# Tangshitao/Semi-supervised-Adaptive-Distillation

Measured on AMD Instinct MI355X. Metric: images/sec (student+teacher fwd + student bwd) R50-FPN distill, 1/2/4/8 MI355X, higher is better.
Workload: dtype f32

## Files before the change

include/ssad_kernels.h:

```cpp
#ifndef SSAD_KERNELS_H_
#define SSAD_KERNELS_H_

#include <stddef.h>
#include <stdint.h>

#ifdef __cplusplus
extern "C" {
#endif

#define SSAD_API __attribute__((visibility("default")))

#define SSAD_E_BADARG (-1)
#define SSAD_E_WORKSPACE (-2)
#define SSAD_MAX_LEVELS 8
#define SSAD_MAX_CONV_PROBLEMS 24
#define SSAD_MAX_POWSUM_INPUTS 8

typedef void* ssad_stream_t;


typedef struct {
  float gamma;
  float alpha;
  float beta;
// ... 226 lines not shown
  float* out;
} ssad_image_norm;
SSAD_API size_t ssad_image_blobs_workspace_bytes(int N, int Hb, int Wb);
SSAD_API int ssad_image_blobs(
    const unsigned char* src, size_t src_bytes, const long long* offset_host, const int* h_host,
    const int* w_host, const int* out_h_host, const int* out_w_host, const double* scale_host,
    const int* flipped_host, int N, int Hb, int Wb, const ssad_image_norm* norms_host, int n_norms,
    void* workspace, size_t workspace_bytes, ssad_stream_t stream);


SSAD_API int ssad_conv_out_size(int in, int kernel, int dilation, int pad_a, int pad_b, int stride);
SSAD_API int ssad_im2col(const float* x, int C, int H, int W, int kh, int kw, int dil_h, int dil_w,
                         int pad_t, int pad_l, int pad_b, int pad_r, int stride_h, int stride_w,
                         float* col, ssad_stream_t stream);
SSAD_API int ssad_im2col_batched(const float* x, int N, int C, int H, int W, int kernel, int stride,
                                 int pad, float* col, ssad_stream_t stream);
SSAD_API int ssad_col2im(const float* col, int C, int H, int W, int kh, int kw, int dil_h,
                         int dil_w, int pad_t, int pad_l, int pad_b, int pad_r, int stride_h,
                         int stride_w, float* x, ssad_stream_t stream);
SSAD_API int ssad_channel_sum(const float* dy, int N, int C, int HW, float* out, int accumulate,
                              ssad_stream_t stream);
SSAD_API int ssad_relu_grad_rowsum(const float* y, const float* dy, float* dx, float* rowsum, int N,
                                   int C, int HW, ssad_stream_t stream);
SSAD_API int ssad_conv1x1_bias_act(const float* x, const float* w, const float* bias,
                                   const float* residual, float* y, int N, int C, int P, int M,
                                   int relu, ssad_stream_t stream);
SSAD_API int ssad_conv1x1_bias_act2(const float* x, int C1, const float* x2, int C2, const float* w,
                                    const float* bias, const float* residual, float* y, int N, int P,
                                    int M, int relu, ssad_stream_t stream);
#define SSAD_GEMM_RELU 1
#define SSAD_GEMM_ACCUMULATE 8
typedef struct ssad_gemm_conv {
  const float* a;
  const float* x;
  float* y;
  const float* bias;
  const float* residual;
  const float* mask;
  int lda, N, K, P, M, flags;
} ssad_gemm_conv;
SSAD_API int ssad_conv1x1_gemm(const ssad_gemm_conv* desc_host, ssad_stream_t stream);
SSAD_API size_t ssad_conv1x1_gemm_split_workspace_bytes(const ssad_gemm_conv* desc_host);
SSAD_API int ssad_conv1x1_gemm_split(const ssad_gemm_conv* desc_host, void* workspace, size_t workspace_bytes,
                                     ssad_stream_t stream);
SSAD_API int ssad_conv1x1_gemm_split_amax(const ssad_gemm_conv* desc_host, const float* packed_a, const unsigned* x_amax,
                                          unsigned* y_amax_out, void* workspace, size_t workspace_bytes,
                                          ssad_stream_t stream);
typedef struct ssad_gemm_pack_entry {
  const float* a;
  float* dst;
  int lda, K, M;
} ssad_gemm_pack_entry;
SSAD_API size_t ssad_gemm_split_filter_floats(int K, int M);
SSAD_API int ssad_gemm_split_pack_filters(const ssad_gemm_pack_entry* entries_host, int n_entries, ssad_stream_t stream);
SSAD_API int ssad_conv_implicit_gemm(const ssad_gemm_conv* d, int C, int H, int W, int kernel, int stride, int pad,
                                     ssad_stream_t stream);
SSAD_API size_t ssad_conv_implicit_gemm_workspace_bytes(int N, int M, int C, int H, int W, int kernel, int stride,
                                                        int pad);
SSAD_API int ssad_conv_implicit_gemm_ws(const ssad_gemm_conv* d, int C, int H, int W, int kernel, int stride, int pad,
                                        void* workspace, size_t workspace_bytes, ssad_stream_t stream);
SSAD_API size_t ssad_conv_kxk_wgrad_workspace_bytes(int N, int C, int H, int W, int M, int kernel, int stride,
                                                    int pad);
SSAD_API int ssad_conv_kxk_wgrad(const float* x, const float* dy, int N, int C, int H, int W, int M, int kernel,
                                 int stride, int pad, float* dw, int accumulate, void* workspace,
                                 size_t workspace_bytes, ssad_stream_t stream);
SSAD_API size_t ssad_conv_kxk_dgrad_workspace_bytes(int N, int C, int H, int W, int M, int kernel, int stride,
                                                    int pad);
SSAD_API int ssad_conv_kxk_dgrad(const float* w, const float* dy, int N, int C, int H, int W, int M, int kernel,
                                 int stride, int pad, float* dx, const float* mask, int accumulate, void* workspace,
                                 size_t workspace_bytes, ssad_stream_t stream);
SSAD_API int ssad_transpose_filter(const float* w, int M, int K, int ldm, float* wt, ssad_stream_t stream);
#define SSAD_MAX_TRANSPOSE_ENTRIES 64
typedef struct ssad_transpose_entry {
  const float* w;
  float* wt;
  int M, K, ldm;
  int reserved;
} ssad_transpose_entry;
SSAD_API int ssad_transpose_filters(const ssad_transpose_entry* entries_host, int n_entries, ssad_stream_t stream);
SSAD_API size_t ssad_conv1x1_wgrad_workspace_bytes(int N, int C, int P, int M);
SSAD_API int ssad_conv1x1_wgrad(const float* x, const float* dy, int N, int C, int P, int M, float* dw,
                                int accumulate, void* workspace, size_t workspace_bytes,
                                ssad_stream_t stream);
SSAD_API size_t ssad_conv1x1_wgrad_split_workspace_bytes(int N, int C, int P, int M);
SSAD_API int ssad_conv1x1_wgrad_split(const float* x, const float* dy, int N, int C, int P, int M, float* dw,
                                      int accumulate, void* workspace, size_t workspace_bytes,
                                      ssad_stream_t stream);
SSAD_API int ssad_conv1x1_wgrad_split_amax(const float* x, const float* dy, int N, int C, int P, int M, float* dw,
                                           int accumulate, void* workspace, size_t workspace_bytes,
                                           const unsigned* x_amax, const unsigned* dy_amax, ssad_stream_t stream);
SSAD_API int ssad_subsample(const float* x, int N, int C, int H, int W, int stride, float* y,
                            ssad_stream_t stream);
SSAD_API int ssad_subsample_grad(const float* dy, int N, int C, int H, int W, int stride, int accumulate,
                                 float* dx, ssad_stream_t stream);
SSAD_API long long ssad_grouped_conv3x3_filter_floats(int C, int group);
SSAD_API int ssad_grouped_conv3x3_pack_filter(const float* w, int C, int group, float* packed,
                                              ssad_stream_t stream);
SSAD_API int ssad_grouped_conv3x3_forward(const float* x, const float* packed, const float* bias, int N, int C,
                                          int H, int W, int group, int stride, int relu, float* y,
                                          ssad_stream_t stream);
SSAD_API int ssad_max_pool_forward(const float* x, int N, int C, int H, int W, int kh, int kw,
                                   int stride_h, int stride_w, int pad_t, int pad_l, int pad_b,
                                   int pad_r, float* y, ssad_stream_t stream);
SSAD_API int ssad_max_pool3x3s2_bias_relu(const float* x, const float* bias, int N, int C, int H,
                                          int W, int relu, float* y, ssad_stream_t stream);
SSAD_API int ssad_max_pool_backward(const float* x, const float* y, const float* dy, int N, int C,
// ... 203 lines not shown
```

semi-supervised-adaptive-distillation_amd/csrc/kernels/gemm_split.hip:

```cpp
#include <stdlib.h>

#include <mutex>

#include "split_common.h"

namespace {

using namespace ssad_split;

constexpr int PT = 128;
constexpr int MT = 256;
constexpr int HDR = 16;

__host__ __device__ constexpr int cdiv(int a, int b) { return (a + b - 1) / b; }

__global__ __launch_bounds__(kThreads) void gsplit_pack_a_kernel(const float* __restrict__ a, int lda, int K, int M,
                                                                 const unsigned* __restrict__ amax, float* __restrict__ dst) {
  const int KB = (K + 7) >> 3;
  const long long slots = (long long)KB * M;
  const float s = pow2f(15 - split_exponent(amax[0]));
  if (blockIdx.x == 0 && threadIdx.x < HDR) reinterpret_cast<unsigned*>(dst)[threadIdx.x] = threadIdx.x == 0 ? amax[0] : 0u;
  uint4* out = reinterpret_cast<uint4*>(dst + HDR);
  for (long long i = (long long)blockIdx.x * kThreads + threadIdx.x; i < slots; i += (long long)gridDim.x * kThreads) {
    const int m = (int)(i % M), kb = (int)(i / M);
// ... 6 lines not shown
    out[slots + i] = __builtin_bit_cast(uint4, lo);
  }
}

struct GPackTable {
  ssad_gemm_pack_entry e[SSAD_MAX_PACK_ENTRIES];
  int count;
};
__global__ __launch_bounds__(kThreads) void gsplit_zero_kernel(const GPackTable t) {
  for (int i = (int)threadIdx.x; i < t.count * HDR; i += kThreads) reinterpret_cast<unsigned*>(t.e[i / HDR].dst)[i % HDR] = 0u;
}
__global__ __launch_bounds__(kThreads) void gsplit_amax_kernel(const GPackTable t) {
  const ssad_gemm_pack_entry& E = t.e[blockIdx.y];
  unsigned m = 0;
  for (int k = (int)blockIdx.x; k < E.K; k += (int)gridDim.x)
    for (int j = (int)threadIdx.x; j < E.M; j += kThreads) {
      const unsigned a = __float_as_uint(E.a[(long long)k * E.lda + j]) & 0x7fffffffu;
      m = m > a ? m : a;
    }
#pragma unroll
  for (int o = 32; o > 0; o >>= 1) {
    const unsigned other = (unsigned)__shfl_xor((int)m, o, 64);
    m = m > other ? m : other;
  }
  __shared__ unsigned red[kThreads / 64];
  if ((threadIdx.x & 63) == 0) red[threadIdx.x >> 6] = m;
  __syncthreads();
  if (threadIdx.x == 0) {
    for (int w = 1; w < kThreads / 64; ++w) m = m > red[w] ? m : red[w];
    if (m) atomicMax(reinterpret_cast<unsigned*>(E.dst), m);
  }
}
__global__ __launch_bounds__(kThreads) void gsplit_pack_multi_kernel(const GPackTable t) {
  const ssad_gemm_pack_entry& E = t.e[blockIdx.y];
  const int KB = (E.K + 7) >> 3;
  const long long slots = (long long)KB * E.M;
  const float s = pow2f(15 - split_exponent(reinterpret_cast<const unsigned*>(E.dst)[0]));
  uint4* out = reinterpret_cast<uint4*>(E.dst + HDR);
  for (long long i = (long long)blockIdx.x * kThreads + threadIdx.x; i < slots; i += (long long)gridDim.x * kThreads) {
    const int m = (int)(i % E.M), kb = (int)(i / E.M);
    float v[8];
#pragma unroll
    for (int j = 0; j < 8; ++j) v[j] = kb * 8 + j < E.K ? E.a[(long long)(kb * 8 + j) * E.lda + m] : 0.0f;
    half8 hi, lo;
    split8(v, s, hi, lo);
    out[i] = __builtin_bit_cast(uint4, hi);
    out[slots + i] = __builtin_bit_cast(uint4, lo);
  }
}

#ifndef GFLY_ABLATE
#define GFLY_ABLATE 0
#endif
constexpr int FKC = 32;
constexpr int FWG = 512;
constexpr int F_XP = (FKC / 8) * PT * 16;
constexpr int F_WP = (FKC / 8) * MT * 16;
constexpr int F_STAGE = 2 * F_XP + 2 * F_WP;
constexpr int F_LDS = 2 * F_STAGE;

struct FArgs {
  const float* x;
  const float* ap;
  float* y;
  const float* bias;
  const float* residual;
  const float* mask;
  const unsigned* amax;
  unsigned* amax_out;
  int N, K, P, M, relu, accumulate;
  int ptiles, mblocks, items;
};

__global__ __launch_bounds__(FWG, 1) void gemm_fly_kernel(const FArgs q) {
  extern __shared__ __attribute__((aligned(16))) char flds[];
  const int tid = threadIdx.x, lane = tid & 63;
  const int wave = __builtin_amdgcn_readfirstlane(tid >> 6);
  const int wm = wave & 3, wp = wave >> 2;
  const int j = lane & 31, h = lane >> 5;
  const int K = q.K, M = q.M, P = q.P;
  const int KB = (K + 7) >> 3;
  const int nchunks = (K + FKC - 1) / FKC;

  int n, p0, ocb;
  {
    const int it = (int)blockIdx.x;
    const int xcd = it & 7, seq = it >> 3;
    const int mb = seq % q.mblocks;
    const int t = (seq / q.mblocks) * 8 + xcd;
    if (t >= q.N * q.ptiles) return;
    n = t / q.ptiles;
    p0 = (t - n * q.ptiles) * PT;
    ocb = mb * MT;
  }
  const unsigned w_lo_off = (unsigned)((long long)KB * M * 16);
  const __amdgpu_buffer_rsrc_t xrs = uniform_rsrc(q.x, (unsigned)((long long)q.N * K * P * 4));
  const __amdgpu_buffer_rsrc_t wrs = uniform_rsrc(q.ap + HDR, 2u * w_lo_off);
  const float sx = pow2f(15 - split_exponent(q.amax[0]));

  float xv[8];
  f32x4 wv[4];
  const int fpx = tid & (PT - 1), fkg = tid >> 7;
  const int fco = tid & (MT - 1), fkq = tid >> 8;
  const unsigned xbase = p0 + fpx < P ? (unsigned)((((long long)n * K + 8 * fkg) * P + p0 + fpx) * 4) : kOob;
  const int P4 = P * 4;
  auto fetch = [&](int c) {
    const int soff = __builtin_amdgcn_readfirstlane(c * FKC * P4);
#pragma unroll
    for (int e = 0; e < 8; ++e)
      xv[e] = __builtin_bit_cast(float, __builtin_amdgcn_raw_buffer_load_b32(
          xrs, c * FKC + 8 * fkg + e < K ? xbase : kOob, soff + e * P4, 0));
#pragma unroll
    for (int i = 0; i < 2; ++i) {
      const int kb = c * (FKC / 8) + fkq + 2 * i;
      const unsigned vo = (kb < KB && ocb + fco < M) ? (unsigned)((kb * M + ocb + fco) * 16) : kOob;
      wv[2 * i] = __builtin_bit_cast(f32x4, __builtin_amdgcn_raw_buffer_load_b128(wrs, vo, 0, 0));
      wv[2 * i + 1] = __builtin_bit_cast(f32x4, __builtin_amdgcn_raw_buffer_load_b128(wrs, vo, (int)w_lo_off, 0));
    }
  };
  auto put = [&](char* stage) {
    half8 hi, lo;
    split8(xv, sx, hi, lo);
    char* px = stage + (fkg * PT + fpx) * 16;
    *reinterpret_cast<half8*>(px) = hi;
    *reinterpret_cast<half8*>(px + F_XP) = lo;
#pragma unroll
    for (int i = 0; i < 2; ++i) {
      char* pw = stage + 2 * F_XP + ((fkq + 2 * i) * MT + fco) * 16;
      *reinterpret_cast<f32x4*>(pw) = wv[2 * i];
      *reinterpret_cast<f32x4*>(pw + F_WP) = wv[2 * i + 1];
    }
  };

  float16v acc[2][2];
#pragma unroll
  for (int i = 0; i < 2; ++i)
#pragma unroll
    for (int tt = 0; tt < 2; ++tt)
#pragma unroll
      for (int r = 0; r < 16; ++r) acc[i][tt][r] = 0.0f;

  auto step = [&](const char* stage, int st) {
    half8 ah[2], al[2], bh[2], bl[2];
    const int kg = 2 * st + h;
#pragma unroll
    for (int i = 0; i < 2; ++i) {
      const char* pw = stage + 2 * F_XP + (kg * MT + wm * 64 + i * 32 + j) * 16;
      ah[i] = *reinterpret_cast<const half8*>(pw);
      al[i] = *reinterpret_cast<const half8*>(pw + F_WP);
      const char* px = stage + (kg * PT + wp * 64 + i * 32 + j) * 16;
      bh[i] = *reinterpret_cast<const half8*>(px);
      bl[i] = *reinterpret_cast<const half8*>(px + F_XP);
    }
#pragma unroll
    for (int pr = 0; pr < ((GFLY_ABLATE & 8) ? 0 : (GFLY_ABLATE & 4) ? 1 : 3); ++pr)
#pragma unroll
      for (int i = 0; i < 2; ++i)
#pragma unroll
        for (int tt = 0; tt < 2; ++tt)
          acc[i][tt] = __builtin_amdgcn_mfma_f32_32x32x16_f16(pr == 1 ? al[i] : ah[i], pr == 2 ? bl[tt] : bh[tt],
                                                              acc[i][tt], 0, 0, 0);
    if (GFLY_ABLATE & 8) {
#pragma unroll
      for (int i = 0; i < 2; ++i) { acc[i][0][0] += (float)ah[i][0] + (float)al[i][1]; acc[i][1][0] += (float)bh[i][0] + (float)bl[i][1]; }
    }
  };

  fetch(0);
  put(flds);
  fetch(1);
  __syncthreads();
  for (int c = 0; c < nchunks; ++c) {
    const char* stage = flds + (c & 1) * F_STAGE;
    char* other = flds + ((c & 1) ^ 1) * F_STAGE;
    __builtin_amdgcn_sched_barrier(0);
    step(stage, 0);
    if (!(GFLY_ABLATE & 2)) put(other);
    __builtin_amdgcn_sched_barrier(0);
    if (!(GFLY_ABLATE & 1)) fetch(c + 2);
    __builtin_amdgcn_sched_barrier(0);
    step(stage, 1);
    __syncthreads();
  }

  const int oc_w = ocb + wm * 64;
  unsigned pvo[2];
#pragma unroll
  for (int tt = 0; tt < 2; ++tt) {
    const int px = p0 + wp * 64 + 32 * tt + j;
    pvo[tt] = px < P ? (unsigned)((((long long)n * M + 4 * h) * P + px) * 4) : kOob;
  }
  const int e2 = split_exponent(q.amax[0]) + split_exponent(reinterpret_cast<const unsigned*>(q.ap)[0]) - 30;
  const bool one_scale = e2 >= -126 && e2 <= 127;
  const float sc1 = one_scale ? pow2f(e2) : pow2f(split_exponent(q.amax[0]) - 15);
  const float sc2 = one_scale ? 1.0f : pow2f(split_exponent(reinterpret_cast<const unsigned*>(q.ap)[0]) - 15);
  const unsigned ybytes = (unsigned)((long long)q.N * M * P * 4);
  const __amdgpu_buffer_rsrc_t yrs = uniform_rsrc(q.y, ybytes);
  const __amdgpu_buffer_rsrc_t rrs = uniform_rsrc(q.residual ? (const void*)q.residual : (const void*)q.y, q.residual ? ybytes : 0u);
  const __amdgpu_buffer_rsrc_t mrs = uniform_rsrc(q.mask ? (const void*)q.mask : (const void*)q.y, q.mask ? ybytes : 0u);
  const __amdgpu_buffer_rsrc_t brs = uniform_rsrc(q.bias ? (const void*)q.bias : (const void*)q.y, q.bias ? (unsigned)M * 4u : 0u);
  const bool relu = q.relu, has_res = q.residual != nullptr, has_mask = q.mask != nullptr, accum = q.accumulate;
  const bool ragged = (M & 7) != 0;
  unsigned ymax = 0;
#pragma unroll
  for (int i = 0; i < 2; ++i) {
    const int oc0 = oc_w + i * 32;
    float4 bq[4];
#pragma unroll
    for (int g = 0; g < 4; ++g)
      bq[g] = __builtin_bit_cast(float4, __builtin_amdgcn_raw_buffer_load_b128(brs, (unsigned)h * 16u, (oc0 + 8 * g) * 4, 0));
#pragma unroll
    for (int tt = 0; tt < 2; ++tt) {
      float rs[16], mk[16], old[16];
#pragma unroll
      for (int r = 0; r < 16; ++r) {
        const int ch = oc0 + 8 * (r >> 2) + (r & 3);
        const unsigned vo = (ch < M && (!ragged || ch + 4 * h < M)) ? pvo[tt] : kOob;
        rs[r] = has_res ? __builtin_bit_cast(float, __builtin_amdgcn_raw_buffer_load_b32(rrs, vo, ch * P4, 0)) : 0.0f;
        mk[r] = has_mask ? __builtin_bit_cast(float, __builtin_amdgcn_raw_buffer_load_b32(mrs, vo, ch * P4, 0)) : 1.0f;
        old[r] = accum ? __builtin_bit_cast(float, __builtin_amdgcn_raw_buffer_load_b32(yrs, vo, ch * P4, 0)) : 0.0f;
      }
#pragma unroll
      for (int g = 0; g < 4; ++g) {
        if (oc0 + 8 * g >= M) continue;
#pragma unroll
        for (int e = 0; e < 4; ++e) {
          const int r = 4 * g + e;
          float v = one_scale ? fmaf(acc[i][tt][r], sc1, bq[g][e]) : acc[i][tt][r] * sc1 * sc2 + bq[g][e];
          v += rs[r];
          if (relu) v = fmaxf(v, 0.0f);
          if (has_mask) v = mk[r] > 0.0f ? v : 0.0f;
          v += old[r];
          const unsigned vo = (!ragged || oc0 + 8 * g + 4 * h + e < M) ? pvo[tt] : kOob;
          __builtin_amdgcn_raw_buffer_store_b32(__builtin_bit_cast(unsigned, v), yrs, vo, (oc0 + 8 * g + e) * P4, 0);
          const unsigned av = __builtin_bit_cast(unsigned, v) & 0x7fffffffu;
          if (vo != kOob) ymax = ymax > av ? ymax : av;
        }
      }
    }
  }
  if (q.amax_out) {
#pragma unroll
    for (int o = 32; o > 0; o >>= 1) {
      const unsigned other = (unsigned)__shfl_xor((int)ymax, o, 64);
      ymax = ymax > other ? ymax : other;
    }
    __syncthreads();
    unsigned* red = reinterpret_cast<unsigned*>(flds);
    if (lane == 0) red[wave] = ymax;
    __syncthreads();
    if (tid == 0) {
      for (int w = 1; w < FWG / 64; ++w) ymax = ymax > red[w] ? ymax : red[w];
      if (ymax) atomicMax(q.amax_out, ymax);
    }
  }
}

constexpr int WT = 256;
constexpr int WPX = 32;
constexpr int W_PL = (WPX / 8) * WT * 16;
constexpr int W_STAGE = 4 * W_PL;
constexpr int W_LDS = 2 * W_STAGE;

struct WPArgs {
  const float* x;
  const float* dy;
  float* slabs;
  const unsigned* xa;
  const unsigned* da;
  int N, C, P, M;
  int mtiles, ctiles, shares, per_share, total, cpi;
  int xcd_runs;
};

__global__ __launch_bounds__(FWG, 1) void wpoint_split_kernel(const WPArgs q) {
  extern __shared__ __attribute__((aligned(16))) char wlds[];
  const int tid = threadIdx.x, lane = tid & 63;
  const int wave = __builtin_amdgcn_readfirstlane(tid >> 6);
  const int wm = wave & 1, wc = wave >> 1;
  const int j = lane & 31, h = lane >> 5;
  const int P = q.P;

  const int tiles = q.mtiles * q.ctiles;
  int share, tile;
  if (q.xcd_runs) {
    const int xcd = blockIdx.x & 7, jj = blockIdx.x >> 3;
    share = xcd * q.xcd_runs + jj / tiles;
    tile = jj % tiles;
  } else {
    share = blockIdx.x / tiles;
    tile = blockIdx.x % tiles;
  }
  const int m0 = (tile / q.ctiles) * WT, c0 = (tile % q.ctiles) * WT;
  const int q_begin = share * q.per_share;
  const int q_end = q_begin + q.per_share < q.total ? q_begin + q.per_share : q.total;

  const __amdgpu_buffer_rsrc_t xrs = uniform_rsrc(q.x, (unsigned)((long long)q.N * q.C * P * 4));
  const __amdgpu_buffer_rsrc_t drs = uniform_rsrc(q.dy, (unsigned)((long long)q.N * q.M * P * 4));
  const float sx = pow2f(15 - split_exponent(q.xa[0]));
  const float sd = pow2f(15 - split_exponent(q.da[0]));

  float dv[2][8], xv[2][8];
  const int fpg = tid & 3, fch = tid >> 2;
  auto fetch = [&](int ck) {
    const int n = __builtin_amdgcn_readfirstlane(ck / q.cpi);
    const int p = (ck - n * q.cpi) * WPX + 8 * fpg;
    const bool pok = ck < q.total && p < P;
#pragma unroll
// ... 99 lines not shown
                                                            float* __restrict__ dw, int accumulate) {
  const long long e = (long long)blockIdx.x * 256 + threadIdx.x;
  if (e >= (long long)M * C) return;
  const int m = (int)(e / C), c = (int)(e - (long long)m * C);
  const float* p = slabs + (long long)m * Cp + c;
  const long long stride = (long long)Mp * Cp;
  float s = 0.0f;
  for (int sh = 0; sh < shares; ++sh) s += p[sh * stride];
  s = (s * pow2f(split_exponent(xa[0]) - 15)) * pow2f(split_exponent(da[0]) - 15);
  dw[e] = accumulate ? dw[e] + s : s;
}

int wpoint_plan(int N, int C, int P, int M, WPArgs* a) {
  if (N <= 0 || C <= 0 || P <= 0 || M <= 0 || (P & 7)) return SSAD_E_BADARG;
  if ((long long)N * C * P * 4 >= (1LL << 31) || (long long)N * M * P * 4 >= (1LL << 31)) return SSAD_E_BADARG;
  a->N = N; a->C = C; a->P = P; a->M = M;
  a->mtiles = cdiv(M, WT); a->ctiles = cdiv(C, WT);
  a->cpi = cdiv(P, WPX);
  a->total = N * a->cpi;
  const int cus = ssad_cu_count(), tiles = a->mtiles * a->ctiles;
  int s = cus / tiles;
  if (s < 1) s = 1;
  if (s >= 8) s &= ~7;
  while (s > 1 && a->total / s < 4) --s;
  a->per_share = cdiv(a->total, s);
  a->shares = cdiv(a->total, a->per_share);
  a->xcd_runs = (a->shares % 8 == 0) ? a->shares / 8 : 0;
  return 0;
}

struct GPlan {
  size_t amax_off, a_off, total;
};
int make_plan(const ssad_gemm_conv* d, GPlan* p) {
  if (!d || d->N <= 0 || d->K <= 0 || d->P <= 0 || d->M <= 0 || d->lda < d->M) return SSAD_E_BADARG;
  const int KB = (d->K + 7) >> 3;
  const long long aslots = (long long)KB * d->M;
  if ((long long)d->N * d->K * d->P * 4 >= (1LL << 31) || (long long)d->N * d->M * d->P * 4 >= (1LL << 31) ||
      aslots * 32 >= (1LL << 31))
    return SSAD_E_BADARG;
  p->amax_off = 0;
  p->a_off = 256;
  p->total = p->a_off + (size_t)HDR * 4 + (size_t)aslots * 32;
  return 0;
}

}

extern "C" {

size_t ssad_conv1x1_gemm_split_workspace_bytes(const ssad_gemm_conv* d) {
  GPlan p;
  return make_plan(d, &p) ? 0 : p.total;
}

size_t ssad_gemm_split_filter_floats(int K, int M) {
  if (K <= 0 || M <= 0) return 0;
  return (size_t)HDR + (size_t)((K + 7) >> 3) * M * 8;
}

int ssad_gemm_split_pack_filters(const ssad_gemm_pack_entry* entries_host, int n_entries, ssad_stream_t stream_) {
  hipStream_t stream = (hipStream_t)stream_;
  if (!entries_host || n_entries < 0) return SSAD_E_BADARG;
  for (int base = 0; base < n_entries; base += SSAD_MAX_PACK_ENTRIES) {
    GPackTable t;
    const int cnt = n_entries - base < SSAD_MAX_PACK_ENTRIES ? n_entries - base : SSAD_MAX_PACK_ENTRIES;
    long long most = 0;
    for (int i = 0; i < cnt; ++i) {
      t.e[i] = entries_host[base + i];
      if (!t.e[i].a || !t.e[i].dst || t.e[i].K <= 0 || t.e[i].M <= 0 || t.e[i].lda < t.e[i].M) return SSAD_E_BADARG;
      const long long slots = (long long)((t.e[i].K + 7) >> 3) * t.e[i].M;
      if (slots > most) most = slots;
    }
    t.count = cnt;
    hipLaunchKernelGGL(gsplit_zero_kernel, dim3(1), dim3(kThreads), 0, stream, t);
    hipLaunchKernelGGL(gsplit_amax_kernel, dim3(64u, (unsigned)cnt), dim3(kThreads), 0, stream, t);
    long long bx = (most + kThreads - 1) / kThreads;
    if (bx > 256) bx = 256;
    hipLaunchKernelGGL(gsplit_pack_multi_kernel, dim3((unsigned)bx, (unsigned)cnt), dim3(kThreads), 0, stream, t);
  }
  return (int)hipGetLastError();
}

int ssad_conv1x1_gemm_split(const ssad_gemm_conv* d, void* workspace, size_t workspace_bytes, ssad_stream_t stream_) {
  return ssad_conv1x1_gemm_split_amax(d, nullptr, nullptr, nullptr, workspace, workspace_bytes, stream_);
}

int ssad_conv1x1_gemm_split_amax(const ssad_gemm_conv* d, const float* packed_a, const unsigned* x_amax,
                                 unsigned* y_amax_out, void* workspace, size_t workspace_bytes, ssad_stream_t stream_) {
  hipStream_t stream = (hipStream_t)stream_;
  GPlan p;
  const int rc = make_plan(d, &p);
  if (rc) return rc;
  if (!d->a || !d->x || !d->y) return SSAD_E_BADARG;
  if ((d->flags & SSAD_GEMM_ACCUMULATE) && (d->bias || d->residual)) return SSAD_E_BADARG;
  if (!workspace || workspace_bytes < p.total) return SSAD_E_WORKSPACE;
  char* ws = (char*)workspace;
  unsigned* amax = (unsigned*)(ws + p.amax_off);
  float* apk = (float*)(ws + p.a_off);
  const int KB = (d->K + 7) >> 3;
  AmaxTable at;
  for (int l = 0; l < kMaxLv; ++l) { at.x[l] = nullptr; at.n[l] = 0; at.block_start[l] = 0; }
  at.count = 2;
  at.amax = amax;
  at.x[0] = d->x; at.n[0] = (long long)d->N * d->K * d->P;
  at.x[1] = d->a; at.n[1] = (long long)d->K * d->lda;
  int blocks = 0;
  for (int l = 0; l < 2; ++l) {
    at.block_start[l] = blocks;
    long long nb = (at.n[l] / 4 + kThreads * 32 - 1) / (kThreads * 32);
    blocks += (int)(nb < 1 ? 1 : nb > 512 ? 512 : nb);
  }
  for (int l = 2; l <= kMaxLv; ++l) at.block_start[l] = blocks;
  if (x_amax && packed_a) {
  } else {
    if (x_amax) { at.n[0] = 0; }
    if (packed_a) { at.n[1] = 0; }
    (void)hipMemsetAsync(amax, 0, 256, stream);
    hipLaunchKernelGGL(split_absmax_kernel, dim3((unsigned)blocks), dim3(kThreads), 0, stream, at);
    if (!packed_a) {
      long long bx = ((long long)KB * d->M + kThreads - 1) / kThreads;
      if (bx > 1024) bx = 1024;
      hipLaunchKernelGGL(gsplit_pack_a_kernel, dim3((unsigned)bx), dim3(kThreads), 0, stream, d->a, d->lda, d->K, d->M,
                         (const unsigned*)(amax + 1), apk);
    }
  }
  FArgs f;
  f.x = d->x; f.ap = packed_a ? packed_a : apk; f.y = d->y; f.bias = d->bias; f.residual = d->residual; f.mask = d->mask;
  f.amax = x_amax ? x_amax : amax;
  f.amax_out = y_amax_out;
  f.N = d->N; f.K = d->K; f.P = d->P; f.M = d->M;
  f.relu = (d->flags & SSAD_GEMM_RELU) ? 1 : 0;
  f.accumulate = (d->flags & SSAD_GEMM_ACCUMULATE) ? 1 : 0;
  f.ptiles = cdiv(d->P, PT);
  f.mblocks = cdiv(d->M, MT);
  const long long tiles = (long long)d->N * f.ptiles;
  if (tiles * f.mblocks >= (1LL << 30)) return SSAD_E_BADARG;
  f.items = (int)(cdiv((int)tiles, 8) * 8 * f.mblocks);
  static std::once_flag lds_once;
  std::call_once(lds_once, [&] {
    (void)hipFuncSetAttribute((const void*)gemm_fly_kernel, hipFuncAttributeMaxDynamicSharedMemorySize, F_LDS);
  });
  hipLaunchKernelGGL(gemm_fly_kernel, dim3((unsigned)f.items), dim3(FWG), F_LDS, stream, f);
  return (int)hipGetLastError();
}

int ssad_split_absmax(const float* x, long long n, unsigned* word, ssad_stream_t stream_) {
  if (!x || !word || n <= 0) return SSAD_E_BADARG;
  AmaxTable at;
  for (int l = 0; l < kMaxLv; ++l) { at.x[l] = nullptr; at.n[l] = 0; at.block_start[l] = 0; }
  at.count = 1;
  at.amax = word;
  at.x[0] = x; at.n[0] = n;
  long long nb = (n / 4 + kThreads * 32 - 1) / (kThreads * 32);
  const int blocks = (int)(nb < 1 ? 1 : nb > 512 ? 512 : nb);
  for (int l = 1; l <= kMaxLv; ++l) at.block_start[l] = blocks;
  hipLaunchKernelGGL(split_absmax_kernel, dim3((unsigned)blocks), dim3(kThreads), 0, (hipStream_t)stream_, at);
  return (int)hipGetLastError();
}

size_t ssad_conv1x1_wgrad_split_workspace_bytes(int N, int C, int P, int M) {
  WPArgs a;
  if (wpoint_plan(N, C, P, M, &a)) return 0;
  return 256 + sizeof(float) * (size_t)a.shares * a.mtiles * WT * a.ctiles * WT;
}

int ssad_conv1x1_wgrad_split(const float* x, const float* dy, int N, int C, int P, int M, float* dw, int accumulate,
                             void* workspace, size_t workspace_bytes, ssad_stream_t stream_) {
  return ssad_conv1x1_wgrad_split_amax(x, dy, N, C, P, M, dw, accumulate, workspace, workspace_bytes, nullptr, nullptr,
                                       stream_);
}

int ssad_conv1x1_wgrad_split_amax(const float* x, const float* dy, int N, int C, int P, int M, float* dw, int accumulate,
                                  void* workspace, size_t workspace_bytes, const unsigned* x_amax,
                                  const unsigned* dy_amax, ssad_stream_t stream_) {
  hipStream_t stream = (hipStream_t)stream_;
  if ((x_amax == nullptr) != (dy_amax == nullptr)) return SSAD_E_BADARG;
  WPArgs a;
  const int rc = wpoint_plan(N, C, P, M, &a);
  if (rc) return rc;
  if (!x || !dy || !dw) return SSAD_E_BADARG;
  const size_t need = 256 + sizeof(float) * (size_t)a.shares * a.mtiles * WT * a.ctiles * WT;
  if (!workspace || workspace_bytes < need) return SSAD_E_WORKSPACE;
  unsigned* amax = (unsigned*)workspace;
  a.x = x; a.dy = dy;
  a.xa = x_amax ? x_amax : amax;
  a.da = dy_amax ? dy_amax : amax + 1;
  a.slabs = (float*)((char*)workspace + 256);
  if (!x_amax) {
  AmaxTable at;
  for (int l = 0; l < kMaxLv; ++l) { at.x[l] = nullptr; at.n[l] = 0; at.block_start[l] = 0; }
  at.count = 2;
  at.amax = amax;
  at.x[0] = x; at.n[0] = (long long)N * C * P;
  at.x[1] = dy; at.n[1] = (long long)N * M * P;
  int blocks = 0;
// ... 22 lines not shown
```

semi-supervised-adaptive-distillation_amd/kernels.py:

```python
import ctypes as C
import os

import torch

_HERE = os.path.dirname(os.path.abspath(__file__))
LIB_NAME = "libcaffe2_detectron_ops_hip.so"
LIB_PATH = os.path.join(_HERE, LIB_NAME)

MAX_LEVELS = 8
CONV_RELU = 1
CONV_MASK_AUX = 2
CONV_SIGMOID = 4
CONV_SPLIT_TAIL = 8


class KernelError(RuntimeError):
    pass


class DistillParams(C.Structure):
    _fields_ = [("gamma", C.c_float), ("alpha", C.c_float), ("beta", C.c_float),
                ("num_classes", C.c_int), ("ignored_label", C.c_int),
                ("scale", C.c_float)]

# ... 160 lines not shown
    L.ssad_conv3x3_forward_f16_levels.argtypes = [C.POINTER(F16Level), i32, vp, vp, i32, i32, i32, vp]
    L.ssad_conv3x3_wgrad_f16_workspace_bytes.restype = sz
    L.ssad_conv3x3_wgrad_f16_workspace_bytes.argtypes = [i32, i32, i32, i32, i32]
    L.ssad_conv3x3_wgrad_f16.argtypes = [vp, vp, i32, i32, i32, i32, i32, i32, f32, vp, vp, vp, sz, vp]
    L.ssad_conv3x3_wgrad_f16_levels_workspace_bytes.restype = sz
    L.ssad_conv3x3_wgrad_f16_levels_workspace_bytes.argtypes = [C.POINTER(F16WgradLevel), i32, i32, i32]
    L.ssad_conv3x3_wgrad_f16_levels.argtypes = [C.POINTER(F16WgradLevel), i32, i32, i32, i32, f32, vp, vp,
                                                vp, sz, vp]
    L.ssad_momentum_sgd_update.argtypes = [vp, vp, vp, vp, f32, f32, i32, i64, vp]
    L.ssad_momentum_sgd_flat.argtypes = [vp, vp, vp, vp, f32, f32, C.POINTER(SgdSegment), i32, vp, vp]
    L.ssad_check_finite.argtypes = [vp, i64, vp, vp]
    L.ssad_loss_scale_update.argtypes = [vp, vp, f32, f32, i32, f32, f32, vp]
    L.ssad_conv_wino_pack_filters.argtypes = [C.POINTER(PackEntry), i32, vp]
    L.ssad_conv_packed_filter_floats.restype = sz
    L.ssad_conv_packed_filter_floats.argtypes = [i32, i32]
    L.ssad_conv_pack_filter.argtypes = [vp, i32, i32, vp, vp, vp]
    L.ssad_conv3x3_forward.argtypes = [C.POINTER(ConvLevel), i32, vp, vp, i32, i32, i32, vp]
    L.ssad_conv_wino_filter_floats.restype = sz
    L.ssad_conv_wino_filter_floats.argtypes = [i32, i32]
    L.ssad_conv_wino_pack_filter.argtypes = [vp, i32, i32, vp, vp, vp]
    L.ssad_conv3x3_forward_wino.argtypes = [C.POINTER(ConvLevel), i32, vp, vp, i32, i32, i32, vp]
    L.ssad_conv3x3_forward_wino24.argtypes = [C.POINTER(ConvLevel), i32, vp, vp, i32, i32, i32, vp]
    L.ssad_conv_wino24_filter_floats.restype = sz
    L.ssad_conv_wino24_filter_floats.argtypes = [i32, i32]
    L.ssad_conv_wino24_pack_filters.argtypes = [C.POINTER(PackEntry), i32, vp]
    L.ssad_conv_split_filter_floats.restype = sz
    L.ssad_conv_split_filter_floats.argtypes = [i32, i32]
    L.ssad_conv_split_pack_filters.argtypes = [C.POINTER(PackEntry), i32, vp]
    L.ssad_conv3x3_split_workspace_bytes.restype = sz
    L.ssad_conv3x3_split_workspace_bytes.argtypes = [C.POINTER(ConvLevel), i32, i32]
    L.ssad_conv3x3_split_items.argtypes = [C.POINTER(ConvLevel), i32, i32]
    L.ssad_conv3x3_forward_split.argtypes = [C.POINTER(ConvLevel), i32, vp, vp, i32, i32, i32, vp, sz, vp, vp, vp]
    L.ssad_conv3x3_forward_wino_launches.argtypes = [C.POINTER(ConvLevel), i32]
    L.ssad_conv3x3_forward_wino_launches_for.argtypes = [C.POINTER(ConvLevel), i32, i32, i32, i32]
    L.ssad_conv_wino_split_tail.argtypes = [i32]
    L.ssad_conv3x3_wgrad_workspace_bytes.restype = sz
    L.ssad_conv3x3_wgrad_workspace_bytes.argtypes = [C.POINTER(ConvLevel), i32, i32, i32]
    L.ssad_conv3x3_wgrad.argtypes = [C.POINTER(ConvLevel), i32, vp, vp, i32, i32, i32, vp, sz, vp]
    L.ssad_conv3x3_wgrad_split_workspace_bytes.restype = sz
    L.ssad_conv3x3_wgrad_split_workspace_bytes.argtypes = [C.POINTER(ConvLevel), i32, i32, i32]
    L.ssad_conv3x3_wgrad_split.argtypes = [C.POINTER(ConvLevel), i32, vp, vp, i32, i32, i32, vp, sz, vp]
    L.ssad_conv1x1_gemm.argtypes = [C.POINTER(GemmConv), vp]
    L.ssad_conv1x1_gemm_split_workspace_bytes.restype = sz
    L.ssad_conv1x1_gemm_split_workspace_bytes.argtypes = [C.POINTER(GemmConv)]
    L.ssad_conv1x1_gemm_split.argtypes = [C.POINTER(GemmConv), vp, sz, vp]
    L.ssad_transpose_filter.argtypes = [vp, i32, i32, i32, vp, vp]
    L.ssad_conv1x1_wgrad_workspace_bytes.restype = sz
    L.ssad_conv1x1_wgrad_workspace_bytes.argtypes = [i32, i32, i32, i32]
    L.ssad_conv1x1_wgrad.argtypes = [vp, vp, i32, i32, i32, i32, vp, i32, vp, sz, vp]
    L.ssad_gemm_split_filter_floats.restype = sz
    L.ssad_gemm_split_filter_floats.argtypes = [i32, i32]
    L.ssad_gemm_split_pack_filters.argtypes = [C.POINTER(GemmPackEntry), i32, vp]
    L.ssad_conv1x1_gemm_split_amax.argtypes = [vp, vp, vp, vp, vp, sz, vp]
    L.ssad_split_absmax.argtypes = [vp, C.c_longlong, vp, vp]
    L.ssad_split_absmax_levels.argtypes = [C.POINTER(ConvLevel), i32, i32, i32, vp, vp]
    L.ssad_conv3x3_wgrad_split_amax.argtypes = [C.POINTER(ConvLevel), i32, vp, vp, i32, i32, i32, vp, sz, vp, vp, vp]
    L.ssad_conv1x1_wgrad_split_amax.argtypes = [vp, vp, i32, i32, i32, i32, vp, i32, vp, sz, vp, vp, vp]
    L.ssad_conv1x1_wgrad_split_workspace_bytes.restype = sz
    L.ssad_conv1x1_wgrad_split_workspace_bytes.argtypes = [i32, i32, i32, i32]
    L.ssad_conv1x1_wgrad_split.argtypes = [vp, vp, i32, i32, i32, i32, vp, i32, vp, sz, vp]
    L.ssad_subsample.argtypes = [vp, i32, i32, i32, i32, i32, vp, vp]
    L.ssad_subsample_grad.argtypes = [vp, i32, i32, i32, i32, i32, i32, vp, vp]
    L.ssad_conv_implicit_gemm.argtypes = [C.POINTER(GemmConv), i32, i32, i32, i32, i32, i32, vp]
    L.ssad_transpose_filters.argtypes = [C.POINTER(TransposeEntry), i32, vp]
    L.ssad_f16_pack_filters.argtypes = [C.POINTER(F16PackEntry), i32, vp]
    L.ssad_conv_implicit_gemm_workspace_bytes.restype = sz
    L.ssad_conv_implicit_gemm_workspace_bytes.argtypes = [i32] * 8
    L.ssad_conv_implicit_gemm_ws.argtypes = [C.POINTER(GemmConv), i32, i32, i32, i32, i32, i32, vp, sz, vp]
    L.ssad_conv_kxk_wgrad_workspace_bytes.restype = sz
    L.ssad_conv_kxk_wgrad_workspace_bytes.argtypes = [i32] * 8
    L.ssad_conv_kxk_wgrad.argtypes = [vp, vp, i32, i32, i32, i32, i32, i32, i32, i32, vp, i32, vp, sz, vp]
    L.ssad_conv_kxk_dgrad_workspace_bytes.restype = sz
    L.ssad_conv_kxk_dgrad_workspace_bytes.argtypes = [i32] * 8
    L.ssad_conv_kxk_dgrad.argtypes = [vp, vp, i32, i32, i32, i32, i32, i32, i32, i32, vp, vp, i32, vp, sz, vp]
    L.ssad_grouped_conv3x3_forward.argtypes = [vp, vp, vp, i32, i32, i32, i32, i32, i32, i32, vp, vp]
    L.ssad_grouped_conv3x3_filter_floats.argtypes = [i32, i32]
    L.ssad_grouped_conv3x3_filter_floats.restype = C.c_longlong
    L.ssad_grouped_conv3x3_pack_filter.argtypes = [vp, i32, i32, vp, vp]
    L.ssad_conv1x1_f16.argtypes = [C.POINTER(PwF16), vp]
    L.ssad_pw_f16_filter_halves.restype = sz
    L.ssad_pw_f16_filter_halves.argtypes = [i32, i32]
    L.ssad_pw_f16_pack_filter.argtypes = [vp, i32, i32, vp, vp, vp]
    L.ssad_conv1x1_wgrad_f16_workspace_bytes.restype = sz
    L.ssad_conv1x1_wgrad_f16_workspace_bytes.argtypes = [i32, i32, i32, i32, i32]
    L.ssad_conv1x1_wgrad_f16.argtypes = [vp, vp, i32, i32, i32, i32, i32, i32, f32, vp, vp, vp, vp, sz, vp]
    L.ssad_f16_elementwise.argtypes = [i32, vp, vp, vp, i32, i32, i32, i32, i32, i32, vp]
    L.ssad_f16_subsample.argtypes = [vp, i32, i32, i32, i32, i32, vp, vp]
    L.ssad_stem_pool_f16.argtypes = [vp, vp, i32, i32, i32, i32, vp, vp]
    L.ssad_grouped_conv3x3_f16_filter_halves.restype = sz
    L.ssad_grouped_conv3x3_f16_filter_halves.argtypes = [i32, i32]
    L.ssad_grouped_conv3x3_f16_pack_filter.argtypes = [vp, i32, i32, vp, vp]
    L.ssad_grouped_conv3x3_f16.argtypes = [vp, vp, vp, i32, i32, i32, i32, i32, i32, vp, vp]
    L.ssad_image_blobs_workspace_bytes.restype = sz
    L.ssad_image_blobs_workspace_bytes.argtypes = [i32, i32, i32]
    L.ssad_image_blobs.argtypes = [vp, sz, vp, vp, vp, vp, vp, vp, vp, i32, i32, i32, C.POINTER(ImageNorm), i32,
                                   vp, sz, vp]
    L.ssad_soft_nms_workspace_bytes.restype = sz
    L.ssad_soft_nms_workspace_bytes.argtypes = [i32]
    L.ssad_soft_nms.argtypes = [vp, vp, vp, i32, i32, i32, f32, f32, f32, vp, vp, vp, sz, vp]
    L.ssad_box_voting.argtypes = [vp, vp, i32, vp, vp, vp, i32, i32, f32, i32, f32, vp, vp, vp]
    L.ssad_retinanet_detect_ex_workspace_bytes.restype = sz
    L.ssad_retinanet_detect_ex_workspace_bytes.argtypes = [i32, i32, i32, vp, vp, i32, C.POINTER(DetectPost)]
    L.ssad_kernels_arch.restype = C.c_char_p
    L.ssad_kernels_abi_version.restype = i32
    if L.ssad_kernels_abi_version() != ABI_VERSION:
        raise KernelError("%s has kernel ABI %d, this binding is written against %d (include/ssad_kernels.h): "
# ... 702 lines not shown
    if dW is None:
        dW = torch.empty((Cout, Cin, 3, 3), dtype=torch.float32, device="cuda")
    if db is None and bias_grad:
        db = torch.empty((Cout,), dtype=torch.float32, device="cuda")
    L = lib()
    n = len(xbs)
    arr = (F16WgradLevel * n)()
    for i, (xb, dyb) in enumerate(zip(xbs, dybs)):
        N, CB, H, W, _ = xb.shape
        assert xb.dtype == torch.float16 and dyb.dtype == torch.float16
        assert xb.is_contiguous() and dyb.is_contiguous()
        assert CB == (Cin + 7) // 8 and dyb.shape == (N, (Cout + 7) // 8, H, W, 8)
        arr[i].x, arr[i].dy, arr[i].N, arr[i].H, arr[i].W = xb.data_ptr(), dyb.data_ptr(), N, H, W
    nbytes = L.ssad_conv3x3_wgrad_f16_levels_workspace_bytes(arr, n, Cin, Cout)
    ws = _workspace(nbytes, "wgrad_f16")
    _check(L.ssad_conv3x3_wgrad_f16_levels(arr, n, Cin, Cout, 0, float(scale), _ptr(dW), _ptr(db), _ptr(ws),
                                           nbytes, _stream()), "conv3x3_wgrad_f16_levels")
    return dW, db



GEMM_RELU = 1
GEMM_ACCUMULATE = 8


def transpose_filter(w, out=None):
    M, Kc = w.shape[0], w.shape[1]
    w2 = _f32c(w.reshape(M, Kc), "w")
    ldm = (M + 3) // 4 * 4
    wt = out if out is not None else torch.empty((Kc, ldm), dtype=torch.float32, device="cuda")
    _check(lib().ssad_transpose_filter(_ptr(w2), M, Kc, ldm, _ptr(wt), _stream()), "transpose_filter")
    return wt


def gemm_conv_desc(a, lda, x, y, K, M, bias=None, residual=None, mask=None, relu=False, accumulate=False):
    N = x.shape[0]
    P = x.numel() // max(N * K, 1)
    return GemmConv(a.data_ptr(), x.data_ptr(), y.data_ptr(), bias.data_ptr() if bias is not None else 0,
                    residual.data_ptr() if residual is not None else 0,
                    mask.data_ptr() if mask is not None else 0, lda, N, K, P, M,
                    (GEMM_RELU if relu else 0) | (GEMM_ACCUMULATE if accumulate else 0))


def _run_gemm(d, what, split):
    L = lib()
    if not split:
        _check(L.ssad_conv1x1_gemm(C.byref(d), _stream()), what)
        return
    need = L.ssad_conv1x1_gemm_split_workspace_bytes(C.byref(d))
    ws = torch.empty(max(need, 16), dtype=torch.uint8, device="cuda")
    _check(L.ssad_conv1x1_gemm_split(C.byref(d), _ptr(ws), ws.numel(), _stream()), what + " (split)")


def split_absmax(x, word=None):
    _f32c(x, "x")
    if word is None:
        word = torch.zeros(1, dtype=torch.int32, device="cuda")
    _check(lib().ssad_split_absmax(_ptr(x), x.numel(), _ptr(word), _stream()), "split_absmax")
    return word


def split_absmax_levels(xs, words=None):
    if words is None:
        words = torch.zeros(len(xs), dtype=torch.int32, device="cuda")
    arr = _conv_levels(xs, None, None)
    _check(lib().ssad_split_absmax_levels(arr, len(xs), xs[0].shape[1], 0, _ptr(words), _stream()), "split_absmax_levels")
    return words


def gemm_split_pack_filter(a, lda, Kc, M):
    dst = torch.empty(lib().ssad_gemm_split_filter_floats(Kc, M), dtype=torch.float32, device="cuda")
    tab = (GemmPackEntry * 1)(GemmPackEntry(a.data_ptr(), dst.data_ptr(), lda, Kc, M))
    _check(lib().ssad_gemm_split_pack_filters(tab, 1, _stream()), "gemm_split_pack_filters")
    return dst


def conv1x1_forward_split_amax(x, wt, M, bias=None, residual=None, relu=False, packed_a=None, x_amax=None, y_amax=None):
    _f32c(x, "x"); _f32c(wt, "wt")
    N, Kc, H, W = x.shape
    y = torch.empty((N, M, H, W), dtype=torch.float32, device="cuda")
    d = gemm_conv_desc(wt, wt.shape[1], x, y, Kc, M, bias, residual, None, relu, False)
    L = lib()
    need = L.ssad_conv1x1_gemm_split_workspace_bytes(C.byref(d))
    ws = torch.empty(max(need, 16), dtype=torch.uint8, device="cuda")
    _check(L.ssad_conv1x1_gemm_split_amax(C.byref(d), _ptr(packed_a), _ptr(x_amax), _ptr(y_amax), _ptr(ws), ws.numel(),
                                          _stream()), "conv1x1_gemm_split_amax")
    return y


def conv1x1_forward(x, wt, M, bias=None, residual=None, relu=False, out=None, split=False):
    _f32c(x, "x"); _f32c(wt, "wt")
    N, Kc, H, W = x.shape
    y = out if out is not None else torch.empty((N, M, H, W), dtype=torch.float32, device="cuda")
    d = gemm_conv_desc(wt, wt.shape[1], x, y, Kc, M, bias, residual, None, relu, False)
    _run_gemm(d, "conv1x1_gemm", split)
    return y


def conv1x1_dgrad(dy, w, mask=None, accumulate_into=None, split=False):
    _f32c(dy, "dy")
    N, M, H, W = dy.shape
    Cc = w.shape[1]
    w2 = _f32c(w.reshape(M, Cc), "w")
    dx = accumulate_into if accumulate_into is not None else torch.empty((N, Cc, H, W), dtype=torch.float32,
                                                                     device="cuda")
    d = gemm_conv_desc(w2, Cc, dy, dx, M, Cc, None, None, mask, False, accumulate_into is not None)
# ... 111 lines not shown
```

Measured before the change: 236.4.

## Add 512-wide output tiles and flattened pixel tiling to split-f16 1x1 GEMM kernel

The fused split-precision 1x1 conv GEMM kernel is templated on output-channel tile width, adding a 512-channel variant with a halved K chunk so the larger weight tile fits in LDS. Each X fragment is then reused across four MFMA row blocks per wave, with alternating wave groups loading X per chunk. Pixel tiles are also flattened across the batch (N*P), so small feature maps no longer waste partial 128-pixel tiles per image. The wide variant is chosen only when M divides by 512 and there are enough items to fill the CUs. The trade-off is more accumulator registers per wave and a shallower K pipeline per chunk.

```diff
diff --git a/include/ssad_kernels.h b/include/ssad_kernels.h
--- a/include/ssad_kernels.h
+++ b/include/ssad_kernels.h
@@ -302,6 +302,7 @@
   int lda, K, M;
 } ssad_gemm_pack_entry;
 SSAD_API size_t ssad_gemm_split_filter_floats(int K, int M);
+SSAD_API int ssad_conv1x1_gemm_split_items(int N, int K, int P, int M, int* channels_per_item);
 SSAD_API int ssad_gemm_split_pack_filters(const ssad_gemm_pack_entry* entries_host, int n_entries, ssad_stream_t stream);
 SSAD_API int ssad_conv_implicit_gemm(const ssad_gemm_conv* d, int C, int H, int W, int kernel, int stride, int pad,
                                      ssad_stream_t stream);
diff --git a/semi-supervised-adaptive-distillation_amd/csrc/kernels/gemm_split.hip b/semi-supervised-adaptive-distillation_amd/csrc/kernels/gemm_split.hip
--- a/semi-supervised-adaptive-distillation_amd/csrc/kernels/gemm_split.hip
+++ b/semi-supervised-adaptive-distillation_amd/csrc/kernels/gemm_split.hip
@@ -82,12 +82,21 @@
 #ifndef GFLY_ABLATE
 #define GFLY_ABLATE 0
 #endif
-constexpr int FKC = 32;
 constexpr int FWG = 512;
-constexpr int F_XP = (FKC / 8) * PT * 16;
-constexpr int F_WP = (FKC / 8) * MT * 16;
-constexpr int F_STAGE = 2 * F_XP + 2 * F_WP;
-constexpr int F_LDS = 2 * F_STAGE;
+template <int MTI>
+struct FCfg {
+  static_assert(MTI == 256 || MTI == 512, "item widths of gemm_fly_kernel");
+  static constexpr int KC = MTI == 256 ? 32 : 16;
+  static constexpr int KG = KC / 8;
+  static constexpr int STEPS = KC / 16;
+  static constexpr int XP = KG * PT * 16;
+  static constexpr int WP = KG * MTI * 16;
+  static constexpr int STAGE = 2 * XP + 2 * WP;
+  static constexpr int LDS = 2 * STAGE;
+  static constexpr int IB = MTI / 128;
+  static constexpr int XT = KG * PT;
+  static constexpr int WGS = FWG / MTI;
+};
 
 struct FArgs {
   const float* x;
@@ -99,10 +108,13 @@
   const unsigned* amax;
   unsigned* amax_out;
   int N, K, P, M, relu, accumulate;
-  int ptiles, mblocks, items;
+  int flat;
+  int ptiles, tiles, mblocks, items;
 };
 
+template <int MTI>
 __global__ __launch_bounds__(FWG, 1) void gemm_fly_kernel(const FArgs q) {
+  using C = FCfg<MTI>;
   extern __shared__ __attribute__((aligned(16))) char flds[];
   const int tid = threadIdx.x, lane = tid & 63;
   const int wave = __builtin_amdgcn_readfirstlane(tid >> 6);
@@ -110,19 +122,29 @@
   const int j = lane & 31, h = lane >> 5;
   const int K = q.K, M = q.M, P = q.P;
   const int KB = (K + 7) >> 3;
-  const int nchunks = (K + FKC - 1) / FKC;
-
-  int n, p0, ocb;
+  const int nchunks = (K + C::KC - 1) / C::KC;
+
+  int t, ocb;
   {
     const int it = (int)blockIdx.x;
     const int xcd = it & 7, seq = it >> 3;
     const int mb = seq % q.mblocks;
-    const int t = (seq / q.mblocks) * 8 + xcd;
-    if (t >= q.N * q.ptiles) return;
+    t = (seq / q.mblocks) * 8 + xcd;
+    if (t >= q.tiles) return;
+    ocb = mb * MTI;
+  }
+  const int NP = q.N * P;
+  auto locate = [&](int col, int& n, int& p) -> bool {
+    if (q.flat) {
+      const int g = t * PT + col;
+      n = g / P;
+      p = g - n * P;
+      return g < NP;
+    }
     n = t / q.ptiles;
-    p0 = (t - n * q.ptiles) * PT;
-    ocb = mb * MT;
-  }
+    p = (t - n * q.ptiles) * PT + col;
+    return p < P;
+  };
   const unsigned w_lo_off = (unsigned)((long long)KB * M * 16);
   const __amdgpu_buffer_rsrc_t xrs = uniform_rsrc(q.x, (unsigned)((long long)q.N * K * P * 4));
   const __amdgpu_buffer_rsrc_t wrs = uniform_rsrc(q.ap + HDR, 2u * w_lo_off);
@@ -130,57 +152,80 @@
 
   float xv[8];
   f32x4 wv[4];
-  const int fpx = tid & (PT - 1), fkg = tid >> 7;
-  const int fco = tid & (MT - 1), fkq = tid >> 8;
-  const unsigned xbase = p0 + fpx < P ? (unsigned)((((long long)n * K + 8 * fkg) * P + p0 + fpx) * 4) : kOob;
+  const int xslot = tid & (C::XT - 1);
+  const int fpx = xslot & (PT - 1), fkg = xslot >> 7;
+  const int xgrp = wave / (C::XT / 64);
+  const int fco = tid & (MTI - 1), fkq = tid / MTI;
+  unsigned xbase;
+  {
+    int n, p;
+    xbase = locate(fpx, n, p) ? (unsigned)((((long long)n * K + 8 * fkg) * P + p) * 4) : kOob;
+  }
   const int P4 = P * 4;
+  auto x_mine = [&](int c) { return C::XT == FWG || (c & 1) == xgrp; };
   auto fetch = [&](int c) {
-    const int soff = __builtin_amdgcn_readfirstlane(c * FKC * P4);
-#pragma unroll
-    for (int e = 0; e < 8; ++e)
-      xv[e] = __builtin_bit_cast(float, __builtin_amdgcn_raw_buffer_load_b32(
-          xrs, c * FKC + 8 * fkg + e < K ? xbase : kOob, soff + e * P4, 0));
+    if (x_mine(c)) {
+      const int soff = __builtin_amdgcn_readfirstlane(c * C::KC * P4);
+#pragma unroll
+      for (int e = 0; e < 8; ++e)
+        xv[e] = __builtin_bit_cast(float, __builtin_amdgcn_raw_buffer_load_b32(
+            xrs, c * C::KC + 8 * fkg + e < K ? xbase : kOob, soff + e * P4, 0));
+    }
 #pragma unroll
     for (int i = 0; i < 2; ++i) {
-      const int kb = c * (FKC / 8) + fkq + 2 * i;
+      const int kb = c * C::KG + fkq + C::WGS * i;
       const unsigned vo = (kb < KB && ocb + fco < M) ? (unsigned)((kb * M + ocb + fco) * 16) : kOob;
       wv[2 * i] = __builtin_bit_cast(f32x4, __builtin_amdgcn_raw_buffer_load_b128(wrs, vo, 0, 0));
       wv[2 * i + 1] = __builtin_bit_cast(f32x4, __builtin_amdgcn_raw_buffer_load_b128(wrs, vo, (int)w_lo_off, 0));
     }
   };
-  auto put = [&](char* stage) {
-    half8 hi, lo;
-    split8(xv, sx, hi, lo);
-    char* px = stage + (fkg * PT + fpx) * 16;
-    *reinterpret_cast<half8*>(px) = hi;
-    *reinterpret_cast<half8*>(px + F_XP) = lo;
+  auto put = [&](char* stage, int c) {
+    if (x_mine(c)) {
+      half8 hi, lo;
+      split8(xv, sx, hi, lo);
+      char* px = stage + (fkg * PT + fpx) * 16;
+      *reinterpret_cast<half8*>(px) = hi;
+      *reinterpret_cast<half8*>(px + C::XP) = lo;
+    }
 #pragma unroll
     for (int i = 0; i < 2; ++i) {
-      char* pw = stage + 2 * F_XP + ((fkq + 2 * i) * MT + fco) * 16;
+      char* pw = stage + 2 * C::XP + ((fkq + C::WGS * i) * MTI + fco) * 16;
       *reinterpret_cast<f32x4*>(pw) = wv[2 * i];
-      *reinterpret_cast<f32x4*>(pw + F_WP) = wv[2 * i + 1];
+      *reinterpret_cast<f32x4*>(pw + C::WP) = wv[2 * i + 1];
     }
   };
 
-  float16v acc[2][2];
-#pragma unroll
-  for (int i = 0; i < 2; ++i)
+  float16v acc[C::IB][2];
+#pragma unroll
+  for (int i = 0; i < C::IB; ++i)
 #pragma unroll
     for (int tt = 0; tt < 2; ++tt)
 #pragma unroll
       for (int r = 0; r < 16; ++r) acc[i][tt][r] = 0.0f;
 
-  auto step = [&](const char* stage, int st) {
-    half8 ah[2], al[2], bh[2], bl[2];
+  half8 bh[2], bl[2];
+  auto load_b = [&](const char* stage, int st) {
     const int kg = 2 * st + h;
 #pragma unroll
+    for (int tt = 0; tt < 2; ++tt) {
+      const char* px = stage + (kg * PT + wp * 64 + tt * 32 + j) * 16;
+      bh[tt] = *reinterpret_cast<const half8*>(px);
+      bl[tt] = *reinterpret_cast<const half8*>(px + C::XP);
+    }
+  };
+  auto mma = [&](const char* stage, int st, int ip) {
+    half8 ah[2], al[2];
+    const int kg = 2 * st + h;
+#pragma unroll
     for (int i = 0; i < 2; ++i) {
-      const char* pw = stage + 2 * F_XP + (kg * MT + wm * 64 + i * 32 + j) * 16;
+      const char* pw = stage + 2 * C::XP + (kg * MTI + wm * (32 * C::IB) + (2 * ip + i) * 32 + j) * 16;
       ah[i] = *reinterpret_cast<const half8*>(pw);
-      al[i] = *reinterpret_cast<const half8*>(pw + F_WP);
-      const char* px = stage + (kg * PT + wp * 64 + i * 32 + j) * 16;
-      bh[i] = *reinterpret_cast<const half8*>(px);
-      bl[i] = *reinterpret_cast<const half8*>(px + F_XP);
+      al[i] = *reinterpret_cast<const half8*>(pw + C::WP);
+      if constexpr (C::IB == 2) {
+        const char* px = stage + (kg * PT + wp * 64 + i * 32 + j) * 16;
+        bh[i] = *reinterpret_cast<const half8*>(px);
+        bl[i] = *reinterpret_cast<const half8*>(px + C::XP);
+      }
     }
 #pragma unroll
     for (int pr = 0; pr < ((GFLY_ABLATE & 8) ? 0 : (GFLY_ABLATE & 4) ? 1 : 3); ++pr)
@@ -188,37 +233,45 @@
       for (int i = 0; i < 2; ++i)
 #pragma unroll
         for (int tt = 0; tt < 2; ++tt)
-          acc[i][tt] = __builtin_amdgcn_mfma_f32_32x32x16_f16(pr == 1 ? al[i] : ah[i], pr == 2 ? bl[tt] : bh[tt],
-                                                              acc[i][tt], 0, 0, 0);
+          acc[2 * ip + i][tt] = __builtin_amdgcn_mfma_f32_32x32x16_f16(pr == 1 ? al[i] : ah[i], pr == 2 ? bl[tt] : bh[tt],
+                                                                       acc[2 * ip + i][tt], 0, 0, 0);
     if (GFLY_ABLATE & 8) {
 #pragma unroll
-      for (int i = 0; i < 2; ++i) { acc[i][0][0] += (float)ah[i][0] + (float)al[i][1]; acc[i][1][0] += (float)bh[i][0] + (float)bl[i][1]; }
+      for (int i = 0; i < 2; ++i) {
+        acc[2 * ip + i][0][0] += (float)ah[i][0] + (float)al[i][1];
+        acc[2 * ip + i][1][0] += (float)bh[i][0] + (float)bl[i][1];
+      }
     }
   };
 
   fetch(0);
-  put(flds);
+  put(flds, 0);
   fetch(1);
   __syncthreads();
   for (int c = 0; c < nchunks; ++c) {
-    const char* stage = flds + (c & 1) * F_STAGE;
-    char* other = flds + ((c & 1) ^ 1) * F_STAGE;
+    const char* stage = flds + (c & 1) * C::STAGE;
+    char* other = flds + ((c & 1) ^ 1) * C::STAGE;
     __builtin_amdgcn_sched_barrier(0);
-    step(stage, 0);
-    if (!(GFLY_ABLATE & 2)) put(other);
+    if constexpr (C::IB == 4) load_b(stage, 0);
+    mma(stage, 0, 0);
+    if (!(GFLY_ABLATE & 2)) put(other, c + 1);
     __builtin_amdgcn_sched_barrier(0);
     if (!(GFLY_ABLATE & 1)) fetch(c + 2);
     __builtin_amdgcn_sched_barrier(0);
-    step(stage, 1);
+    if constexpr (C::STEPS == 2) {
+      mma(stage, 1, 0);
+    } else {
+      mma(stage, 0, 1);
+    }
     __syncthreads();
   }
 
-  const int oc_w = ocb + wm * 64;
+  const int oc_w = ocb + wm * (32 * C::IB);
   unsigned pvo[2];
 #pragma unroll
   for (int tt = 0; tt < 2; ++tt) {
-    const int px = p0 + wp * 64 + 32 * tt + j;
-    pvo[tt] = px < P ? (unsigned)((((long long)n * M + 4 * h) * P + px) * 4) : kOob;
+    int n, p;
+    pvo[tt] = locate(wp * 64 + 32 * tt + j, n, p) ? (unsigned)((((long long)n * M + 4 * h) * P + p) * 4) : kOob;
   }
   const int e2 = split_exponent(q.amax[0]) + split_exponent(reinterpret_cast<const unsigned*>(q.ap)[0]) - 30;
   const bool one_scale = e2 >= -126 && e2 <= 127;
@@ -233,7 +286,7 @@
   const bool ragged = (M & 7) != 0;
   unsigned ymax = 0;
 #pragma unroll
-  for (int i = 0; i < 2; ++i) {
+  for (int i = 0; i < C::IB; ++i) {
     const int oc0 = oc_w + i * 32;
     float4 bq[4];
 #pragma unroll
@@ -284,6 +337,33 @@
       if (ymax) atomicMax(q.amax_out, ymax);
     }
   }
+}
+
+int fly_mode() {
+  const char* e = getenv("SSAD_GEMM_FLY_ITEMS");
+  if (!e || !*e) return 1;
+  const int v = atoi(e);
+  return v == 0 ? 0 : v == 2 ? 2 : 1;
+}
+int fly_plan(int N, int P, int M, FArgs* f, int* width) {
+  const int mode = fly_mode();
+  f->flat = mode != 0;
+  f->ptiles = cdiv(P, PT);
+  const long long tiles = f->flat ? ((long long)N * P + PT - 1) / PT : (long long)N * f->ptiles;
+  *width = (mode != 0 && M % 512 == 0 && (mode == 2 || tiles * (M / 512) >= ssad_cu_count())) ? 512 : MT;
+  f->mblocks = cdiv(M, *width);
+  if (tiles * f->mblocks >= (1LL << 30)) return SSAD_E_BADARG;
+  f->tiles = (int)tiles;
+  f->items = cdiv(f->tiles, 8) * 8 * f->mblocks;
+  return 0;
+}
+template <int MTI>
+void launch_fly(const FArgs& f, hipStream_t stream) {
+  static std::once_flag lds_once;
+  std::call_once(lds_once, [&] {
+    (void)hipFuncSetAttribute((const void*)gemm_fly_kernel<MTI>, hipFuncAttributeMaxDynamicSharedMemorySize, FCfg<MTI>::LDS);
+  });
+  hipLaunchKernelGGL(gemm_fly_kernel<MTI>, dim3((unsigned)f.items), dim3(FWG), FCfg<MTI>::LDS, stream, f);
 }
 
 constexpr int WT = 256;
@@ -489,6 +569,17 @@
 size_t ssad_conv1x1_gemm_split_workspace_bytes(const ssad_gemm_conv* d) {
   GPlan p;
   return make_plan(d, &p) ? 0 : p.total;
+}
+
+int ssad_conv1x1_gemm_split_items(int N, int K, int P, int M, int* channels_per_item) {
+  ssad_gemm_conv d = {};
+  d.N = N; d.K = K; d.P = P; d.M = M; d.lda = M;
+  GPlan p;
+  FArgs f;
+  int width = MT;
+  if (make_plan(&d, &p) || fly_plan(N, P, M, &f, &width)) return SSAD_E_BADARG;
+  if (channels_per_item) *channels_per_item = width;
+  return f.items;
 }
 
 size_t ssad_gemm_split_filter_floats(int K, int M) {
@@ -569,16 +660,10 @@
   f.N = d->N; f.K = d->K; f.P = d->P; f.M = d->M;
   f.relu = (d->flags & SSAD_GEMM_RELU) ? 1 : 0;
   f.accumulate = (d->flags & SSAD_GEMM_ACCUMULATE) ? 1 : 0;
-  f.ptiles = cdiv(d->P, PT);
-  f.mblocks = cdiv(d->M, MT);
-  const long long tiles = (long long)d->N * f.ptiles;
-  if (tiles * f.mblocks >= (1LL << 30)) return SSAD_E_BADARG;
-  f.items = (int)(cdiv((int)tiles, 8) * 8 * f.mblocks);
-  static std::once_flag lds_once;
-  std::call_once(lds_once, [&] {
-    (void)hipFuncSetAttribute((const void*)gemm_fly_kernel, hipFuncAttributeMaxDynamicSharedMemorySize, F_LDS);
-  });
-  hipLaunchKernelGGL(gemm_fly_kernel, dim3((unsigned)f.items), dim3(FWG), F_LDS, stream, f);
+  int width = MT;
+  if (fly_plan(d->N, d->P, d->M, &f, &width)) return SSAD_E_BADARG;
+  if (width == 512) launch_fly<512>(f, stream);
+  else launch_fly<256>(f, stream);
   return (int)hipGetLastError();
 }
 
diff --git a/semi-supervised-adaptive-distillation_amd/kernels.py b/semi-supervised-adaptive-distillation_amd/kernels.py
--- a/semi-supervised-adaptive-distillation_amd/kernels.py
+++ b/semi-supervised-adaptive-distillation_amd/kernels.py
@@ -236,6 +236,7 @@
     L.ssad_gemm_split_filter_floats.argtypes = [i32, i32]
     L.ssad_gemm_split_pack_filters.argtypes = [C.POINTER(GemmPackEntry), i32, vp]
     L.ssad_conv1x1_gemm_split_amax.argtypes = [vp, vp, vp, vp, vp, sz, vp]
+    L.ssad_conv1x1_gemm_split_items.argtypes = [i32, i32, i32, i32, C.POINTER(i32)]
     L.ssad_split_absmax.argtypes = [vp, C.c_longlong, vp, vp]
     L.ssad_split_absmax_levels.argtypes = [C.POINTER(ConvLevel), i32, i32, i32, vp, vp]
     L.ssad_conv3x3_wgrad_split_amax.argtypes = [C.POINTER(ConvLevel), i32, vp, vp, i32, i32, i32, vp, sz, vp, vp, vp]
@@ -1044,6 +1045,13 @@
     _check(L.ssad_conv1x1_gemm_split(C.byref(d), _ptr(ws), ws.numel(), _stream()), what + " (split)")
 
 
+def conv1x1_gemm_split_items(N, Kc, P, M):
+    width = C.c_int(0)
+    n = lib().ssad_conv1x1_gemm_split_items(N, Kc, P, M, C.byref(width))
+    _check(min(n, 0), "conv1x1_gemm_split_items")
+    return n, width.value
+
+
 def split_absmax(x, word=None):
     _f32c(x, "x")
     if word is None:
```

Result: no change. 238.2 (median of 6 runs) (+0.8%).
